# bilgili/Libre

Measured on AMD Instinct MI355X. Metric: Msamples/s + frames/s, 1024^3 volume @ 1024^2 viewport, higher is better.
Workload: dtype u8

## Files before the change

include/vrc_hip.h:

```cpp
#ifndef VRC_HIP_H
#define VRC_HIP_H

#include <stddef.h>
#include <stdint.h>

#ifdef __cplusplus
extern "C" {
#endif

#define VRC_OK 0
#define VRC_EINVAL 1
#define VRC_EHIP 2
#define VRC_EFULL 3
#define VRC_ENOMEM 4
#define VRC_EUNSUPPORTED 5
#define VRC_EHIERARCHY 6
#define VRC_ECOMM 7

typedef struct vrc_ctx vrc_ctx;
typedef struct vrc_pool vrc_pool;

typedef struct
{
    float textureMin[3];
// ... 76 lines not shown

#define VRC_OPT_RAY_CACHE 22
#define VRC_OPT_RAY_CACHE_USED 23

#define VRC_OPT_WALK_CACHE 24
#define VRC_WALK_CACHE_ALWAYS 2
#define VRC_OPT_WALK_CACHE_USED 25
#define VRC_OPT_WALK_CACHE_BUDGET 26
#define VRC_OPT_WALK_CACHE_BYTES 27
#define VRC_OPT_WALK_LEAN_USED 28
#define VRC_OPT_SHADING 29
#define VRC_OPT_SHADING_AMBIENT 30
#define VRC_OPT_COMPOSITE_DEPTH 31
#define VRC_OPT_PREINTEGRATION 32
#define VRC_OPT_PREINT_BUILDS 33
#define VRC_OPT_WALK_UNIFORM_ONLY 34
#define VRC_OPT_WALK_UNIFORM_ONLY_USED 35
#define VRC_OPT_STORE_THROUGH 36
#define VRC_OPT_STORE_THROUGH_USED 37
#define VRC_OPT_FIRST_VISIT_TABLE 38
#define VRC_OPT_FIRST_VISIT_TABLE_USED 39
#define VRC_OPT_LEAN_FREE_MARCH 40
#define VRC_OPT_LEAN_FREE_MARCH_USED 41
#define VRC_WALK_CACHE_DEFAULT_BUDGET ( 512ll << 20 )








#define VRC_VARIANT_CUDARAYCASTER 0
#define VRC_VARIANT_GLRAYCASTER 1

#define VRC_FILTER_NEAREST 0
#define VRC_FILTER_TRILINEAR 1

#define VRC_KERNEL_AUTO 0
#define VRC_REFERENCE_ORDER_MAX_NODES 4096
#define VRC_KERNEL_REFERENCE_ORDER 1
#define VRC_KERNEL_GRID_DDA 2
#define VRC_KERNEL_LDS 3
#define VRC_KERNEL_PACKED 5
#define VRC_KERNEL_RAY_LOD 4

// ... 90 lines not shown
```

libre_amd/csrc/vrc_api.hip:

```cpp
#include "../../include/vrc_hip.h"
#include "vrc_internal.h"
#include "vrc_plan.h"
#include "vrc_tables.h"

#include <algorithm>
#include <array>
#include <cmath>
#include <cstdarg>
#include <cstdio>
#include <cstring>
#include <memory>
#include <mutex>
#include <string>
#include <vector>

namespace
{
thread_local std::string g_lastError;

int fail( int code, const std::string& msg )
{
    g_lastError = msg;
    return code;
}
// ... 85 lines not shown

struct vrc_walk_cache
{
    enum { IDLE = 0, COUNTING = 1, VALID = 2 };
    int state = IDLE;
    uint32_t* dLists = nullptr;
    size_t words = 0;
    uint32_t k = 0;
    vrc_walk_count* dMax = nullptr;
    vrc_walk_count* hMax = nullptr;
    hipEvent_t ev = nullptr;
    vrc_frame frame;
    vrc_frame prevFrame;
    bool prevSet = false;
    uint64_t prevGen = 0, gen = 0;
    const uint32_t* slotInfo = nullptr;
    int64_t used = 0;
    bool leanAsked = false, lean = false;
    int64_t leanUsed = 0;
    unsigned long long gathers = 0;
    int64_t uniformUsed = 0;
    int64_t throughUsed = 0;
    int64_t freeUsed = 0;
};

struct vrc_first_visit
{
    void* dTable = nullptr;
    uint64_t gen = 0, prevGen = 0;
    bool grey = false;
    int64_t used = 0;
};

struct vrc_ctx
{
    int device = 0;
    hipStream_t ownStream = nullptr;
    hipStream_t stream = nullptr;
    vrc_options opt;
    vrc_latches latch;

    float* dTf = nullptr;
    float* hTf = nullptr;
    uint64_t tfVersion = 0;
    float planes[6][4];
    uint32_t nPlanes = 0;
// ... 225 lines not shown
        vrc_ctx_destroy( c );
        return fail( VRC_EHIP, msg );
    }
    c->stream = c->ownStream;
    *c->hCounter = 0;
    std::memcpy( c->hTf, tf, sizeof( tf ) );
    c->tfGrey = true;
    if( const char* g = std::getenv( "VRC_GREY_TABLE" ) )
        c->opt.greyTable = g[0] != '0';
    c->tfVersion = 1;
    *out = c;
    return VRC_OK;
}

void vrc_ctx_destroy( vrc_ctx* c )
{
    if( !c )
        return;
    (void)hipSetDevice( c->device );
    if( c->stream ) (void)hipStreamSynchronize( c->stream );
    const std::initializer_list< void* > device = {
        c->dTf,      c->dLut,     c->dPreint,  c->fbOwn,     c->dNodes,    c->dGrid,    c->dTileOrder, c->dRayCache,
        c->walk.dLists, c->walk.dMax, c->dRayList, c->dMipMax, c->dMeanSum, c->dMeanCount, c->dProjOut, c->dMipDepth,
        c->dIsoGrad, c->dDepthOut, c->dRowMap, c->dCounter,  c->dFrameHist, c->dHistRefs, c->first.dTable };
    const std::initializer_list< void* > pinned = { c->hTf, c->hStage, c->walk.hMax, c->hCounter, c->hFrameHist, c->hHistRefs };
    for( void* d : device )
        if( d ) (void)hipFree( d );
    for( void* h : pinned )
        if( h ) (void)hipHostFree( h );
    for( hipEvent_t e : c->stageEvent )
        if( e ) (void)hipEventDestroy( e );
    for( hipEvent_t e : c->histRefsEvent )
        if( e ) (void)hipEventDestroy( e );
    if( c->walk.ev ) (void)hipEventDestroy( c->walk.ev );
    c->evRing.reset();
    if( c->ownStream ) (void)hipStreamDestroy( c->ownStream );
    delete c;
}

int vrc_ctx_set_stream( vrc_ctx* c, void* s )
{
    if( !c )
        return fail( VRC_EINVAL, "vrc_ctx_set_stream: ctx is NULL" );
    VRC_HIP_CHECK( hipSetDevice( c->device ) );
    VRC_HIP_CHECK( hipStreamSynchronize( c->stream ) );
    c->stream = s ? (hipStream_t)s : c->ownStream;
    c->waitedPoolUid = c->waitedGen = 0;
// ... 59 lines not shown
    case VRC_OPT_WALK_UNIFORM_ONLY_USED:
        return fail( VRC_EINVAL, "vrc_set_option: VRC_OPT_WALK_UNIFORM_ONLY_USED is read-only" );
    case VRC_OPT_STORE_THROUGH:
        if( value != 0 && value != 1 )
            return fail( VRC_EINVAL, "vrc_set_option: VRC_OPT_STORE_THROUGH is 0 (plain stores) or 1 (write-through)" );
        c->opt.storeThrough = value;
        return VRC_OK;
    case VRC_OPT_STORE_THROUGH_USED:
        return fail( VRC_EINVAL, "vrc_set_option: VRC_OPT_STORE_THROUGH_USED is read-only" );
    case VRC_OPT_FIRST_VISIT_TABLE:
        if( value != 0 && value != 1 )
            return fail( VRC_EINVAL, "vrc_set_option: VRC_OPT_FIRST_VISIT_TABLE is 0 (march every visit) or 1 (first visits from the table)" );
        c->opt.firstVisitTable = value;
        return VRC_OK;
    case VRC_OPT_FIRST_VISIT_TABLE_USED:
        return fail( VRC_EINVAL, "vrc_set_option: VRC_OPT_FIRST_VISIT_TABLE_USED is read-only" );
    case VRC_OPT_LEAN_FREE_MARCH:
        if( value != 0 && value != 1 )
            return fail( VRC_EINVAL, "vrc_set_option: VRC_OPT_LEAN_FREE_MARCH is 0 (every visit tests for the exit) or 1 (not where it is out of reach)" );
        c->opt.leanFreeMarch = value;
        return VRC_OK;
    case VRC_OPT_LEAN_FREE_MARCH_USED:
        return fail( VRC_EINVAL, "vrc_set_option: VRC_OPT_LEAN_FREE_MARCH_USED is read-only" );
    case VRC_OPT_PROJECTION:
        if( value != VRC_PROJECTION_COMPOSITE && value != VRC_PROJECTION_MIP && value != VRC_PROJECTION_ISO )
            return fail( VRC_EINVAL, "vrc_set_option: VRC_OPT_PROJECTION is 0 (composite), 1 (maximum intensity) or 2 (isosurface)" );
        if( value == VRC_PROJECTION_ISO && !c->isoSet )
            return fail( VRC_EINVAL, "vrc_set_option: VRC_OPT_PROJECTION = VRC_PROJECTION_ISO needs vrc_set_isosurface first" );
        c->opt.projection = value;
        return VRC_OK;
    case VRC_OPT_MIP_SKIP: c->opt.mipSkip = value ? 1 : 0; return VRC_OK;
    case VRC_OPT_MIP_FOLD:
        if( value != VRC_MIP_FOLD_MAX && value != VRC_MIP_FOLD_MIN && value != VRC_MIP_FOLD_MEAN )
            return fail( VRC_EINVAL, "vrc_set_option: VRC_OPT_MIP_FOLD is 0 (maximum), 1 (minimum) or 2 (mean)" );
        c->opt.mipFold = value;
        return VRC_OK;
    case VRC_OPT_MIP_DEPTH:
        if( value != 0 && value != 1 )
            return fail( VRC_EINVAL, "vrc_set_option: VRC_OPT_MIP_DEPTH is 0 (off) or 1 (keep the depth of the projected sample)" );
        c->opt.mipDepth = value;
        return VRC_OK;
    case VRC_OPT_MIP_DEPTH_CUE:
        if( value < 0 || value > 1000 )
            return fail( VRC_EINVAL, "vrc_set_option: VRC_OPT_MIP_DEPTH_CUE is the cue strength in thousandths, 0 (off) to 1000" );
        c->opt.mipDepthCue = value;
        return VRC_OK;
// ... 48 lines not shown
    case VRC_OPT_STEPPING: *value = c->opt.stepping; return VRC_OK;
    case VRC_OPT_KERNEL_TIMING: *value = c->opt.timing; return VRC_OK;
    case VRC_OPT_DEPTH_SPLIT: *value = c->opt.depthSplit; return VRC_OK;
    case VRC_OPT_ERT_COMPACTION: *value = c->opt.ertParts; return VRC_OK;
    case VRC_OPT_GREY_TABLE: *value = c->opt.greyTable; return VRC_OK;
    case VRC_OPT_PACKED_ATLAS: *value = c->opt.packedAtlas; return VRC_OK;
    case VRC_OPT_UNIFORM_BRICKS: *value = c->opt.uniformBricks; return VRC_OK;
    case VRC_OPT_STREAM_MARKERS: *value = c->opt.streamMarkers; return VRC_OK;
    case VRC_OPT_RAY_CACHE: *value = c->opt.rayCache; return VRC_OK;
    case VRC_OPT_RAY_CACHE_USED: *value = c->rayCacheUsed; return VRC_OK;
    case VRC_OPT_WALK_CACHE: *value = c->opt.walkCache; return VRC_OK;
    case VRC_OPT_WALK_CACHE_USED: *value = c->walk.used; return VRC_OK;
    case VRC_OPT_WALK_CACHE_BUDGET: *value = c->opt.walkBudget; return VRC_OK;
    case VRC_OPT_WALK_CACHE_BYTES: *value = (int64_t)( c->walk.words * sizeof( uint32_t ) ); return VRC_OK;
    case VRC_OPT_WALK_LEAN_USED: *value = c->walk.leanUsed; return VRC_OK;
    case VRC_OPT_WALK_UNIFORM_ONLY: *value = c->opt.walkUniformOnly; return VRC_OK;
    case VRC_OPT_WALK_UNIFORM_ONLY_USED: *value = c->walk.uniformUsed; return VRC_OK;
    case VRC_OPT_STORE_THROUGH: *value = c->opt.storeThrough; return VRC_OK;
    case VRC_OPT_STORE_THROUGH_USED: *value = c->walk.throughUsed; return VRC_OK;
    case VRC_OPT_FIRST_VISIT_TABLE: *value = c->opt.firstVisitTable; return VRC_OK;
    case VRC_OPT_FIRST_VISIT_TABLE_USED: *value = c->first.used; return VRC_OK;
    case VRC_OPT_LEAN_FREE_MARCH: *value = c->opt.leanFreeMarch; return VRC_OK;
    case VRC_OPT_LEAN_FREE_MARCH_USED: *value = c->walk.freeUsed; return VRC_OK;
    case VRC_OPT_PROJECTION: *value = c->opt.projection; return VRC_OK;
    case VRC_OPT_MIP_SKIP: *value = c->opt.mipSkip; return VRC_OK;
    case VRC_OPT_MIP_FOLD: *value = c->opt.mipFold; return VRC_OK;
    case VRC_OPT_MIP_DEPTH: *value = c->opt.mipDepth; return VRC_OK;
    case VRC_OPT_MIP_DEPTH_CUE: *value = c->opt.mipDepthCue; return VRC_OK;
    case VRC_OPT_VARIANT: *value = c->opt.variant; return VRC_OK;
    case VRC_OPT_SHADING: *value = c->opt.shading; return VRC_OK;
    case VRC_OPT_SHADING_AMBIENT: *value = c->opt.shadingAmbient; return VRC_OK;
    case VRC_OPT_COMPOSITE_DEPTH: *value = c->opt.compositeDepth; return VRC_OK;
    case VRC_OPT_PREINTEGRATION: *value = c->opt.preint; return VRC_OK;
    case VRC_OPT_PREINT_BUILDS: *value = c->preintBuilds; return VRC_OK;
    case VRC_OPT_KERNEL_USED: *value = c->stats.kernel_variant; return VRC_OK;
    case VRC_OPT_GRID_WALK_USED: *value = c->gridWalkUsed; return VRC_OK;
    default: return fail( VRC_EINVAL, "vrc_get_option: unknown option" );
    }
}

int vrc_set_ray_lod( vrc_ctx* c, int enable, float screenSpaceError, float worldSpacePerPixel )
{
    if( !c )
        return fail( VRC_EINVAL, "vrc_set_ray_lod: ctx is NULL" );
    if( enable && ( !( screenSpaceError > 0.0f ) || !( worldSpacePerPixel > 0.0f ) ) )
        return fail( VRC_EINVAL, "vrc_set_ray_lod: screen-space error and world space per pixel must be > 0" );
// ... 855 lines not shown
{
    if( !c )
        return fail( VRC_EINVAL, "vrc_get_framebuffer: ctx is NULL" );
    VRC_TRY( resolve_clear( c ) );
    if( deviceRgba ) *deviceRgba = ctx_fb( c );
    if( width ) *width = c->fbW;
    if( height ) *height = c->fbH;
    return VRC_OK;
}

struct render_pass
{
    const vrc_view_data* view;
    const vrc_node_data* nodes;
    uint32_t nNodes;
    const vrc_render_data* render;
    vrc_pool* pool;
    vrc_lut_params lp;
    vrc_mode mode;
    vrc_form form;
    bool sameNodes, tableWalk;
    size_t pixels, plane;
    bool walkCount, walkRecord;
    vrc_raycast_args a;
};

static int render_check_args( vrc_ctx* c, const vrc_view_data* view, const vrc_node_data* nodes, uint32_t nNodes,
                              const vrc_render_data* render, vrc_pool* pool )
{
    if( !c || !view || !render || !pool )
        return fail( VRC_EINVAL, "vrc_render: NULL argument" );
    if( nNodes > 0 && !nodes )
        return fail( VRC_EINVAL, "vrc_render: nodes is NULL" );
    if( pool->device != c->device )
        return fail( VRC_EINVAL, "vrc_render: pool lives on another device" );
    if( !ctx_fb( c ) || c->fbW == 0 )
        return fail( VRC_EINVAL, "vrc_render: vrc_pre_render has not been called" );
    if( view->glViewport[2] != c->fbW ||
        ( c->rowMap.empty() ? view->glViewport[3] : (uint32_t)c->rowMap.size() ) != c->fbH )
        return fail( VRC_EINVAL, "vrc_render: viewport differs from the pixel buffer" );
    if( render->samplesPerRay == 0 )
        return fail( VRC_EINVAL, "vrc_render: samplesPerRay is 0" );
    if( render->dataSourceRange[1] == render->dataSourceRange[0] )
        return fail( VRC_EINVAL, "vrc_render: empty data source range" );
    return VRC_OK;
}
// ... 487 lines not shown
    }
    else if( p.walkCount )
        f.walkLean = leanAsked ? 1u : 0u;
    w.throughUsed = vrc_plan_store_through( c->opt, w.used, f.width, f.height ) ? 1 : 0;
    f.storeThrough = (uint32_t)w.throughUsed;
    vrc_first_visit& fv = c->first;
    const bool grey = p.a.greyTable;
    vrc_first_visit_facts k = { w.used, f.walkLean, f.clearFirst != 0u, p.mode.classify,
                                fv.gen != 0u && fv.gen == c->lutGen && fv.grey == grey };
    if( vrc_plan_first_visit_build( c->opt, k, fv.prevGen == c->lutGen ) )
    {
        if( !fv.dTable )
            VRC_HIP_CHECK( hipMalloc( &fv.dTable, (size_t)VRC_FIRST_VISIT_ENTRIES * VRC_FIRST_VISIT_ROWS * sizeof( vrc_f4 ) ) );
        VRC_HIP_CHECK( vrc_launch_build_first_visit( c->dLut, fv.dTable, grey, c->stream ) );
        fv.gen = c->lutGen;
        fv.grey = grey;
        k.current = true;
    }
    fv.prevGen = c->lutGen;
    fv.used = vrc_plan_first_visit( c->opt, k ) ? 1 : 0;
    f.firstVisit = fv.used ? fv.dTable : nullptr;
    w.freeUsed = vrc_plan_lean_free_march( c->opt, w.used, f.walkLean, p.mode.classify ) ? 1 : 0;
    f.leanFree = (uint32_t)w.freeUsed;
    return VRC_OK;
}

static int render_march( vrc_ctx* c, render_pass& p )
{
    vrc_raycast_args& a = p.a;
    vrc_frame& f = a.frame;
    const vrc_mode& m = p.mode;
    VRC_TRY( ctx_wait_uploads( c, p.pool ) );
    if( p.walkCount )
    {
        VRC_HIP_CHECK( hipMemsetAsync( c->walk.dMax, 0, sizeof( vrc_walk_count ), c->stream ) );
        VRC_HIP_CHECK( vrc_launch_walk_record( a, c->walk.dMax, c->stream ) );
        VRC_HIP_CHECK( hipMemcpyAsync( c->walk.hMax, c->walk.dMax, sizeof( vrc_walk_count ), hipMemcpyDeviceToHost, c->stream ) );
        VRC_HIP_CHECK( hipEventRecord( c->walk.ev, c->stream ) );
        std::memcpy( &c->walk.frame, &f, sizeof( f ) );
        c->walk.state = vrc_walk_cache::COUNTING;
        f.walkLean = 0u;
    }
    if( p.walkRecord )
    {
        VRC_HIP_CHECK( vrc_launch_walk_record( a, nullptr, c->stream ) );
        c->walk.state = vrc_walk_cache::VALID;
        f.walkCache = nullptr;
        f.walkPlane = f.walkK = 0u;
        f.walkLean = f.walkSlots = 0u;
    }
    if( c->opt.count )
        VRC_HIP_CHECK( hipMemsetAsync( c->dCounter, 0, sizeof( unsigned long long ), c->stream ) );
    if( c->opt.timing && c->evUsed == c->evRing->pairs.size() )
    {
        if( c->evRing->pairs.size() >= 4096 )
        {
            VRC_HIP_CHECK( hipEventSynchronize( c->evRing->pairs[c->evUsed - 1].second ) );
            for( size_t i = 0; i < c->evUsed; ++i )
            {
                float ms = 0.f;
                VRC_HIP_CHECK( hipEventElapsedTime( &ms, c->evRing->pairs[i].first, c->evRing->pairs[i].second ) );
                c->evFoldedMs += ms;
            }
            c->evFoldedLaunches += (uint32_t)c->evUsed;
            c->evUsed = 0;
        }
        else
        {
            hipEvent_t a0 = nullptr, a1 = nullptr;
            VRC_HIP_CHECK( hipEventCreate( &a0 ) );
            VRC_HIP_CHECK( hipEventCreate( &a1 ) );
            c->evRing->pairs.push_back( { a0, a1 } );
// ... 346 lines not shown
```

libre_amd/csrc/vrc_core.h:

```cpp
#ifndef VRC_CORE_H
#define VRC_CORE_H

#if !defined( VRC_DEV_BUILD ) && ( \
    defined( VRC_ABLATE_NO_FETCH ) || \
    defined( VRC_WG_TIMELINE ) || \
    defined( VRC_UNIFORM_GROUP ) || \
    defined( VRC_LEAN_GROUP ) || defined( VRC_LEAN_FREE_GROUP ) || \
    defined( VRC_TEST_BIAS_ENTRY ) || \
    defined( VRC_LDS_STATS ) || defined( VRC_LDS_STATS2 ) || \
    defined( VRC_LDS_TIMING ) || \
    defined( VRC_LDS_PASSES ) || defined( VRC_LDS_ROWS ) || defined( VRC_LDS_OCC ) || defined( VRC_LDS_STAGE_N ) || \
    defined( VRC_LDS_ROWS16 ) || defined( VRC_LDS_OCC16 ) || defined( VRC_LDS_STAGE_N16 ) || \
    defined( VRC_LDS_KMAX ) || \
    defined( VRC_LDS_MAX_DZ ) || \
    defined( VRC_LDS_LBATCH ) || \
    defined( VRC_LDS_GBATCH ) || \
    defined( VRC_LDS_G ) || defined( VRC_LDS_GF ) || \
    defined( VRC_LDS_WAVES ) || \
    defined( VRC_LDS_REFILL ) || defined( VRC_LDS_SOON ) || \
    defined( VRC_GROUP ) || \
    defined( VRC_GREY_GROUP ) || \
    defined( VRC_GREY_MAX_WAVES ) || defined( VRC_REPLAY_GREY_MAX_WAVES ) || \
    defined( VRC_REPLAY_UNIFORM_MAX_WAVES ) || defined( VRC_REPLAY_UNIFORM_WG_WAVES ) || \
    defined( VRC_LGROUP ) || \
// ... 111 lines not shown
    uint32_t* meanCount;
    float* mipDepth;
    float mipCue;
    float* rayCache;
    uint32_t rayCachePlane;
    uint32_t rayMode;
    float* isoGrad;
    uint32_t isoThreshold;
    float isoStored;
    float isoClassify;
    float isoAmbient;
    uint32_t* walkCache;
    uint32_t walkPlane;
    uint32_t walkK;
#define VRC_WALK_LEAN_UNIFORM 2u
    uint32_t walkLean;
    uint32_t walkSlots;
    float shadeAmbient;
    float cdepthTau;
    const vrc_f4* preintTable;
    uint32_t storeThrough;
    const void* firstVisit;
    uint32_t leanFree;
};
#define VRC_RAY_COMPUTE 0u
#define VRC_RAY_STORE 1u
#define VRC_RAY_LOAD 2u
#define VRC_RAY_CACHE_PLANES 10u

struct vrc_layout
{
    uint32_t slots[3];
    uint32_t slotDim[3];
};

VRC_HD uint32_t vrc_mb_y( uint32_t u ) { return ( ( u & 3u ) << 3 ) | ( ( u & 4u ) << 5 ); }
VRC_HD uint32_t vrc_mb_z( uint32_t u ) { return ( ( u & 3u ) << 5 ) | ( ( u & 4u ) << 6 ); }
#define VRC_MB_FIX_Y( u ) ( 96u * ( ( ( u ) >> 2 ) & 1u ) )
#define VRC_MB_FIX_Z( u ) ( 32u * ( ( u ) & 3u ) )
struct vrc_lay
{
    uint32_t a, b, c;
};
VRC_HD vrc_lay vrc_make_lay( uint32_t sbx, uint32_t sby )
{
    vrc_lay l;
// ... 4118 lines not shown
VRC_HD vrc_f4 vrc_lean_narrow( const vrc_f4& c, const vrc_f4* ) { return c; }
VRC_HD vrc_f4 vrc_lean_widen( const vrc_f2& c ) { return vrc_f4{ c.x, c.x, c.x, c.w }; }
VRC_HD vrc_f4 vrc_lean_widen( const vrc_f4& c ) { return c; }
VRC_HD uint32_t vrc_lean_slot_load( const vrc_frame& f, uint32_t packed )
{
    const uint32_t idx = packed & ( ( 1u << VRC_WALK_LEAN_INDEX_BITS ) - 1u );
    const bool have = f.slotInfo != nullptr;
    const uint32_t* const from = have ? f.slotInfo : f.walkCache;
    const uint32_t last = have ? f.walkSlots - 1u : 0u;
    const uint32_t i = idx != 0u ? idx - 1u : 0u;
    return from[i < last ? i : last];
}
VRC_HD uint32_t vrc_lean_slot_word( const vrc_frame& f, uint32_t packed, uint32_t loaded )
{
    return ( f.slotInfo != nullptr && ( packed & ( ( 1u << VRC_WALK_LEAN_INDEX_BITS ) - 1u ) ) != 0u ) ? loaded : 0u;
}
VRC_HD uint32_t vrc_lean_list_word( const vrc_frame& f, uint32_t rayIndex, uint32_t v )
{
    const uint32_t lastVisit = f.walkK - 1u;
    const size_t plane = 2u + 4u * (size_t)( v < lastVisit ? v : lastVisit );
    return f.walkCache[(size_t)rayIndex + plane * f.walkPlane];
}

template < bool COUNT, int MODE, int GROUP, bool UNIFORM_ONLY = false >
VRC_HD void vrc_pixel_walk_replay_lean( const vrc_frame& f, const vrc_dev_node* __restrict__ nodes,
                                        const uint8_t* __restrict__ atlas, const vrc_f4* lut, const vrc_classifier& cls,
                                        vrc_f4* __restrict__ pixelBuffer, uint32_t px, uint32_t py, uint32_t& nSamples,
                                        uint32_t rayIndex )
{
    typedef typename vrc_lean_colour< MODE >::type E;
    (void)cls;
    const E* const tab = reinterpret_cast< const E* >( lut );
    const uint32_t pixelPos = py * f.width + px;
    const vrc_f4 zero = { 0.f, 0.f, 0.f, 0.f };
    const uint32_t listed = f.walkCache[rayIndex];
    const uint32_t count = listed < f.walkK ? listed : f.walkK;
    if( count == 0u )
    {
        if( f.clearFirst )
            vrc_store_pixel( f, pixelBuffer, pixelPos, zero );
        return;
    }
    const vrc_f4 start = f.clearFirst ? zero : pixelBuffer[pixelPos];
    if( start.w > VRC_EARLY_EXIT )
        return;
    E color = vrc_lean_narrow( start, (const E*)nullptr );
    const uint32_t lastNode = f.nodeCount - 1u;
    const bool freeMarch = f.leanFree != 0u;
    uint32_t packed = vrc_lean_list_word( f, rayIndex, 0u );
    uint32_t packedNext = vrc_lean_list_word( f, rayIndex, 1u );
    uint32_t loaded = vrc_lean_slot_load( f, packed );
    uint32_t k = 0u;
    bool ended = false;
    if constexpr( !COUNT )
// ... 456 lines not shown
```

libre_amd/csrc/vrc_internal.h:

```cpp
#ifndef VRC_INTERNAL_H
#define VRC_INTERNAL_H

#include <hip/hip_runtime.h>
#include <hip/hip_ext.h>
#include <stdint.h>

#include "vrc_core.h"

#ifndef VRC_TILE_W
#define VRC_TILE_W 8u
#endif
#define VRC_TILE_H ( 64u / VRC_TILE_W )

#define VRC_NO_TILE 0xFFFFFFFFu
#define VRC_WAVES_PER_GROUP 4u
#ifndef VRC_SUPER_UNITS
#define VRC_SUPER_UNITS 1u
#endif
#define VRC_XCDS 8u
__host__ __device__ inline uint32_t vrc_super_x( uint32_t tilesX ) { return ( ( tilesX + 1u ) / 2u + VRC_SUPER_UNITS - 1u ) / VRC_SUPER_UNITS; }
__host__ __device__ inline uint32_t vrc_schedule_units( uint32_t tilesX, uint32_t tilesY )
{
    const uint32_t nSuper = vrc_super_x( tilesX ) * vrc_super_x( tilesY );
    return ( nSuper + VRC_XCDS - 1u ) / VRC_XCDS * VRC_XCDS * VRC_SUPER_UNITS * VRC_SUPER_UNITS;
// ... 111 lines not shown
#endif
#ifndef VRC_SMALL_GROUP
#define VRC_SMALL_GROUP 24
#endif
#ifndef VRC_SMALL_LAUNCH_TILES
#define VRC_SMALL_LAUNCH_TILES 6144u
#endif
static inline bool vrc_walk_replay_eligible( const vrc_raycast_args& a )
{
    return a.gridDda && a.gridTable && !a.packed && !a.linear && a.elemBytes == 1 && !a.bigAtlas && !a.clamp &&
           a.fixedStepping && a.ertParts <= 1 && !a.depthSplit && !a.shade && !a.cdepth && !a.preint && VRC_TILE_W == 8u;
}
static inline int vrc_walk_replay_group( const vrc_raycast_args& a )
{
    const uint32_t tiles = ( ( a.frame.width + VRC_TILE_W - 1 ) / VRC_TILE_W ) * ( ( a.frame.height + VRC_TILE_H - 1 ) / VRC_TILE_H );
    return tiles <= VRC_SMALL_LAUNCH_TILES ? VRC_SMALL_GROUP : ( a.greyTable ? VRC_GREY_GROUP : VRC_GROUP );
}
struct vrc_walk_count
{
    uint32_t longest, notLean;
    unsigned long long visits, gathers;
};
hipError_t vrc_launch_walk_record( const vrc_raycast_args& a, vrc_walk_count* result, hipStream_t stream );
hipError_t vrc_launch_raycast_replay( const vrc_raycast_args& a, hipStream_t stream );

hipError_t vrc_launch_raycast_mip( const vrc_raycast_args& a, hipStream_t stream );
hipError_t vrc_launch_raycast_minip( const vrc_raycast_args& a, hipStream_t stream );
hipError_t vrc_launch_raycast_meanip( const vrc_raycast_args& a, hipStream_t stream );

struct vrc_projection_state
{
    const uint32_t* mipMax;
    const unsigned long long* meanSum;
    const uint32_t* meanCount;
    uint32_t pixels;
    uint32_t fold;
    uint32_t floatState;
    float shift;
};
hipError_t vrc_launch_projection_values( const vrc_projection_state& st, float* values, uint32_t* counts, hipStream_t stream );

hipError_t vrc_launch_raycast_mip_depth( const vrc_raycast_args& a, int fold, hipStream_t stream );
hipError_t vrc_launch_projection_depths( const vrc_frame& f, const float* depth, uint32_t pixels, float* t, float* xyz,
                                         hipStream_t stream );

hipError_t vrc_launch_raycast_iso( const vrc_raycast_args& a, hipStream_t stream );
// ... 23 lines not shown
```

libre_amd/csrc/vrc_kernels_walk.hip:

```cpp
#include "vrc_internal.h"

#define VRC_WALK_WAVES VRC_WAVES_PER_GROUP
#define VRC_WALK_THREADS ( 64u * VRC_WALK_WAVES )

__device__ inline void vrc_walk_lane_pixel( uint32_t tile, uint32_t tilesX, uint32_t lane, uint32_t& px, uint32_t& py )
{
    const uint32_t tx = tile % tilesX, ty = tile / tilesX;
    const uint32_t lx = ( lane & 1u ) | ( ( lane >> 1 ) & 2u ) | ( ( lane >> 2 ) & 4u );
    const uint32_t ly = ( ( lane >> 1 ) & 1u ) | ( ( lane >> 2 ) & 2u ) | ( ( lane >> 3 ) & 4u );
    px = tx * 8u + lx;
    py = ty * 8u + ly;
}

__global__ __launch_bounds__( VRC_WALK_THREADS ) void vrc_k_walk_record(
    const vrc_frame f, const vrc_dev_node* __restrict__ nodes, const int32_t* __restrict__ gridTable,
    vrc_walk_count* __restrict__ result, const uint32_t tilesX, const uint32_t nTiles )
{
    const uint32_t lane = threadIdx.x & 63u;
    const uint32_t tile = blockIdx.x * VRC_WALK_WAVES + ( threadIdx.x >> 6 );
    if( tile >= nTiles )
        return;
    uint32_t px, py;
    vrc_walk_lane_pixel( tile, tilesX, lane, px, py );
    const uint32_t rayIndex = tile * 64u + lane;
// ... 38 lines not shown
                        0, stream, a.frame, a.nodes, a.gridTable, result, tilesX, nTiles );
    return hipGetLastError();
}

template < typename E >
__global__ __launch_bounds__( 64 ) void vrc_k_build_first_visit( const vrc_f4* __restrict__ lut, E* __restrict__ table, const E start )
{
    const uint32_t e = blockIdx.x * 64u + threadIdx.x;
    if( e < VRC_FIRST_VISIT_ENTRIES )
        vrc_first_visit_row< E >( table + (size_t)e * VRC_FIRST_VISIT_ROWS, vrc_lean_narrow( lut[e], (const E*)nullptr ), start );
}

hipError_t vrc_launch_build_first_visit( const vrc_f4* lut, void* table, bool grey, hipStream_t stream )
{
    if( !lut || !table )
        return hipErrorInvalidValue;
    const dim3 grid( ( VRC_FIRST_VISIT_ENTRIES + 63u ) / 64u ), block( 64 );
    if( grey )
        hipLaunchKernelGGL( vrc_k_build_first_visit< vrc_f2 >, grid, block, 0, stream, lut, static_cast< vrc_f2* >( table ),
                            vrc_f2{ 0.f, 0.f } );
    else
        hipLaunchKernelGGL( vrc_k_build_first_visit< vrc_f4 >, grid, block, 0, stream, lut, static_cast< vrc_f4* >( table ),
                            vrc_f4{ 0.f, 0.f, 0.f, 0.f } );
    return hipGetLastError();
}

#ifndef VRC_REPLAY_GREY_MAX_WAVES
#define VRC_REPLAY_GREY_MAX_WAVES 6
#endif
#ifndef VRC_REPLAY_UNIFORM_MAX_WAVES
#define VRC_REPLAY_UNIFORM_MAX_WAVES 8
#endif
#ifndef VRC_REPLAY_UNIFORM_WG_WAVES
#define VRC_REPLAY_UNIFORM_WG_WAVES VRC_WALK_WAVES
#endif
#define VRC_REPLAY_K_MIN_WAVES ( UNIFORM ? VRC_REPLAY_UNIFORM_MAX_WAVES : ( GROUP > VRC_GREY_GROUP ? 2 : 5 ) )
#define VRC_REPLAY_K_MAX_WAVES \
    ( UNIFORM ? VRC_REPLAY_UNIFORM_MAX_WAVES \
              : ( GROUP > VRC_GREY_GROUP ? 8 : ( MODE == VRC_MODE_GREY ? VRC_REPLAY_GREY_MAX_WAVES : 5 ) ) )
#define VRC_REPLAY_K_WAVES ( UNIFORM ? VRC_REPLAY_UNIFORM_WG_WAVES : VRC_WALK_WAVES )
template < bool COUNT, int MODE, int GROUP, bool LEAN = false, bool UNIFORM = false >
__global__ __launch_bounds__( 64u * VRC_REPLAY_K_WAVES ) __attribute__( ( amdgpu_waves_per_eu( VRC_REPLAY_K_MIN_WAVES, VRC_REPLAY_K_MAX_WAVES ) ) ) void vrc_k_raycast_replay(
    const vrc_frame f, const vrc_dev_node* __restrict__ nodes, const uint8_t* __restrict__ atlas,
    const vrc_f4* __restrict__ lutGlobal, const vrc_classifier cls, vrc_f4* __restrict__ pixelBuffer,
    unsigned long long* __restrict__ sampleCounter, const uint32_t* __restrict__ tileOrder, const uint32_t tilesX,
    const uint32_t nTiles )
// ... 9 lines not shown
        vrc_f2* const lut2 = reinterpret_cast< vrc_f2* >( lut );
        for( uint32_t i = tid; i < VRC_LUT_ENTRIES; i += THREADS )
        {
            const vrc_f4 e = lutGlobal[i];
            lut2[i] = vrc_f2{ e.x, e.w };
        }
    }
    else
    {
        for( uint32_t i = tid; i < VRC_TFP_ENTRIES; i += THREADS )
            lut[i] = lutGlobal[i];
    }
    if constexpr( !UNIFORM )
    {
        const vrc_lay lay = vrc_make_lay( f.sbx, f.sby );
        for( uint32_t u = tid; u < 256u; u += THREADS )
        {
            vrc_addr_tab[u] = vrc_lay_x( lay, u );
            vrc_addr_tab[256u + u] = vrc_lay_y( lay, u );
            vrc_addr_tab[512u + u] = vrc_lay_z( lay, u );
        }
    }
    __syncthreads();
    const uint32_t slotIndex = blockIdx.x * WAVES + ( tid >> 6 );
    const uint32_t tilesY = nTiles / tilesX;
    if( slotIndex >= vrc_schedule_slots( tilesX, tilesY ) )
        return;
    const uint32_t tile = vrc_slot_tile( tileOrder, slotIndex, tilesX, tilesY );
    if( tile == VRC_NO_TILE )
        return;
    uint32_t px, py;
    vrc_walk_lane_pixel( tile, tilesX, lane, px, py );

    uint32_t nSamples = 0;
    if( px < f.width && py < f.height )
    {
        if constexpr( LEAN )
            vrc_pixel_walk_replay_lean< COUNT, MODE, GROUP, UNIFORM >( f, nodes, atlas, lut, cls, pixelBuffer, px, py,
                                                                       nSamples, tile * 64u + lane );
        else
            vrc_pixel_walk_replay< COUNT, MODE, GROUP >( f, nodes, atlas, lut, cls, pixelBuffer, px, py, nSamples,
                                                         tile * 64u + lane );
    }
    if( COUNT )
    {
        unsigned long long s = nSamples;
#pragma unroll
        for( int off = 32; off > 0; off >>= 1 )
            s += __shfl_down( s, off, 64 );
        if( lane == 0 && s != 0 )
            atomicAdd( sampleCounter, s );
    }
}

template < bool COUNT, int MODE, int GROUP, bool LEAN, bool UNIFORM = false >
// ... 43 lines not shown
```

libre_amd/csrc/vrc_plan.h:

```cpp
#ifndef VRC_PLAN_H
#define VRC_PLAN_H

#include "../../include/vrc_hip.h"

struct vrc_options
{
    int64_t kernel = VRC_KERNEL_AUTO, variant = VRC_VARIANT_CUDARAYCASTER;
    int64_t filter = 0, tfFracBits = 8, stepping = 1;
    int64_t count = 0, timing = 1, streamMarkers = 0;
    int64_t depthSplit = 0, ertParts = 0;
    int64_t packedAtlas = 1, uniformBricks = 1, greyTable = 1, tileOrder = 1, rayCache = 1;
    int64_t walkCache = 1, walkBudget = VRC_WALK_CACHE_DEFAULT_BUDGET, walkUniformOnly = 1;
    int64_t projection = VRC_PROJECTION_COMPOSITE, mipSkip = 1, mipFold = VRC_MIP_FOLD_MAX;
    int64_t mipDepth = 0, mipDepthCue = 0;
    int64_t shading = 0, shadingAmbient = 250;
    int64_t compositeDepth = 0, preint = 0;
    int64_t storeThrough = 1;
    int64_t firstVisitTable = 1;
    int64_t leanFreeMarch = 1;
};

struct vrc_latches
{
    int64_t projection = -1, fold = -1, depth = -1, cue = -1;
    bool iso = false;
    float isoValue = 0.0f, isoAmbient = 0.0f;
    int64_t shading = -1, shadingAmbient = -1, compositeDepth = -1, preint = -1;
};

struct vrc_refusal
{
    int code;
    const char* msg;
};

struct vrc_mode
{
    bool iso = false, mip = false;
    bool mipDepth = false, mean = false;
    bool shade = false, cdepth = false, preint = false;
    bool linear = false;
    bool classify = false;
// ... 203 lines not shown
    uint32_t walkLean;
    bool clearFirst;
    bool classify;
    bool current;
};
inline bool vrc_plan_first_visit_wanted( const vrc_options& o, const vrc_first_visit_facts& k )
{
    return o.firstVisitTable != 0 && k.walkUsed == 4 && k.walkLean != 0u && k.clearFirst && !k.classify && o.count == 0;
}
inline bool vrc_plan_first_visit( const vrc_options& o, const vrc_first_visit_facts& k )
{
    return vrc_plan_first_visit_wanted( o, k ) && k.current;
}
inline bool vrc_plan_first_visit_build( const vrc_options& o, const vrc_first_visit_facts& k, bool prevSameGeneration )
{
    return vrc_plan_first_visit_wanted( o, k ) && !k.current && prevSameGeneration;
}

inline bool vrc_plan_lean_free_march( const vrc_options& o, int64_t walkUsed, uint32_t walkLean, bool classify )
{
    return o.leanFreeMarch != 0 && walkUsed == 4 && walkLean != 0u && !classify && o.count == 0;
}

#endif
```

libre_amd/vrc.py:

```python
import ctypes as C
import os

_HERE = os.path.dirname(os.path.abspath(__file__))
LIB_PATH = os.path.join(_HERE, "lib", "libvrc_hip.so")

VRC_OK, VRC_EINVAL, VRC_EHIP, VRC_EFULL, VRC_ENOMEM, VRC_EUNSUPPORTED, VRC_EHIERARCHY, VRC_ECOMM = range(8)
OPT_KERNEL, OPT_FILTER, OPT_TF_FRAC_BITS, OPT_COUNT_SAMPLES, OPT_TILE_ORDER, OPT_STEPPING, OPT_VARIANT, OPT_KERNEL_USED, OPT_KERNEL_TIMING, OPT_DEPTH_SPLIT, OPT_ERT_COMPACTION, OPT_GREY_TABLE, OPT_PACKED_ATLAS, OPT_GRID_WALK_USED, OPT_UNIFORM_BRICKS = range(1, 16)
OPT_PROJECTION, OPT_MIP_SKIP, OPT_MIP_FOLD = 16, 17, 18
OPT_MIP_DEPTH, OPT_MIP_DEPTH_CUE = 19, 20
OPT_STREAM_MARKERS = 21
OPT_RAY_CACHE, OPT_RAY_CACHE_USED = 22, 23
OPT_WALK_CACHE, OPT_WALK_CACHE_USED, OPT_WALK_CACHE_BUDGET, OPT_WALK_CACHE_BYTES = 24, 25, 26, 27
WALK_CACHE_ALWAYS = 2
OPT_WALK_LEAN_USED = 28
OPT_SHADING, OPT_SHADING_AMBIENT = 29, 30
OPT_COMPOSITE_DEPTH = 31
OPT_PREINTEGRATION = 32
OPT_PREINT_BUILDS = 33
OPT_WALK_UNIFORM_ONLY, OPT_WALK_UNIFORM_ONLY_USED = 34, 35
OPT_STORE_THROUGH, OPT_STORE_THROUGH_USED = 36, 37
OPT_FIRST_VISIT_TABLE, OPT_FIRST_VISIT_TABLE_USED = 38, 39
OPT_LEAN_FREE_MARCH, OPT_LEAN_FREE_MARCH_USED = 40, 41
PREINT_VALUE, PREINT_TEXEL = 0, 1
PROJECTION_COMPOSITE, PROJECTION_MIP, PROJECTION_ISO = 0, 1, 2
MIP_FOLD_MAX, MIP_FOLD_MIN, MIP_FOLD_MEAN = 0, 1, 2
VARIANT_CUDARAYCASTER, VARIANT_GLRAYCASTER = 0, 1
FILTER_NEAREST, FILTER_TRILINEAR = 0, 1
KERNEL_AUTO, KERNEL_REFERENCE_ORDER, KERNEL_GRID_DDA, KERNEL_LDS, KERNEL_RAY_LOD, KERNEL_PACKED = 0, 1, 2, 3, 4, 5

VOXEL_UINT8, VOXEL_UINT16, VOXEL_UINT32, VOXEL_INT8, VOXEL_INT16, VOXEL_INT32, VOXEL_FLOAT32 = range(7)

ABI_VERSION = 4

f32x3 = C.c_float * 3
u32x3 = C.c_uint32 * 3


class NodeData(C.Structure):
    _fields_ = [("textureMin", f32x3), ("textureSize", f32x3),
                ("aabbMin", f32x3), ("aabbSize", f32x3)]


class ViewData(C.Structure):
    _fields_ = [("eyePosition", f32x3), ("glViewport", C.c_uint32 * 4),
                ("invProjMatrix", C.c_float * 16), ("modelViewMatrix", C.c_float * 16),
# ... 156 lines not shown
```

Baseline: 14.20 million.

## Precompute resolved per-visit walk words for uniform-only lean replay

Adds a resolve kernel that, once per walk-cache generation, folds each ray's list word and slot-info lookup into a single resolved word (sample count, one-value flag, value byte). The uniform-only lean replay then reads these words directly with prefetching, which removes the indirect slot-table loads and dependent address math from the per-frame replay. Tile and slot indices are also made wave-uniform through readfirstlane. The cost is an extra device buffer of K words per pixel, a one-time resolve pass, and invalidation bookkeeping tied to generation and slot info.

```diff
diff --git a/include/vrc_hip.h b/include/vrc_hip.h
--- a/include/vrc_hip.h
+++ b/include/vrc_hip.h
@@ -122,6 +122,8 @@
 #define VRC_OPT_FIRST_VISIT_TABLE_USED 39
 #define VRC_OPT_LEAN_FREE_MARCH 40
 #define VRC_OPT_LEAN_FREE_MARCH_USED 41
+#define VRC_OPT_WALK_RESOLVED 42
+#define VRC_OPT_WALK_RESOLVED_USED 43
 #define VRC_WALK_CACHE_DEFAULT_BUDGET ( 512ll << 20 )
 
 
diff --git a/libre_amd/csrc/vrc_api.hip b/libre_amd/csrc/vrc_api.hip
--- a/libre_amd/csrc/vrc_api.hip
+++ b/libre_amd/csrc/vrc_api.hip
@@ -131,6 +131,12 @@
     int64_t uniformUsed = 0;
     int64_t throughUsed = 0;
     int64_t freeUsed = 0;
+    uint32_t* dResolved = nullptr;
+    size_t resolvedWords = 0;
+    bool resolvedValid = false;
+    uint64_t resolvedGen = 0;
+    const uint32_t* resolvedSlotInfo = nullptr;
+    int64_t resolvedUsed = 0;
 };
 
 struct vrc_first_visit
@@ -402,7 +408,8 @@
     const std::initializer_list< void* > device = {
         c->dTf,      c->dLut,     c->dPreint,  c->fbOwn,     c->dNodes,    c->dGrid,    c->dTileOrder, c->dRayCache,
         c->walk.dLists, c->walk.dMax, c->dRayList, c->dMipMax, c->dMeanSum, c->dMeanCount, c->dProjOut, c->dMipDepth,
-        c->dIsoGrad, c->dDepthOut, c->dRowMap, c->dCounter,  c->dFrameHist, c->dHistRefs, c->first.dTable };
+        c->dIsoGrad, c->dDepthOut, c->dRowMap, c->dCounter,  c->dFrameHist, c->dHistRefs, c->first.dTable,
+        c->walk.dResolved };
     const std::initializer_list< void* > pinned = { c->hTf, c->hStage, c->walk.hMax, c->hCounter, c->hFrameHist, c->hHistRefs };
     for( void* d : device )
         if( d ) (void)hipFree( d );
@@ -508,6 +515,13 @@
         return VRC_OK;
     case VRC_OPT_LEAN_FREE_MARCH_USED:
         return fail( VRC_EINVAL, "vrc_set_option: VRC_OPT_LEAN_FREE_MARCH_USED is read-only" );
+    case VRC_OPT_WALK_RESOLVED:
+        if( value != 0 && value != 1 )
+            return fail( VRC_EINVAL, "vrc_set_option: VRC_OPT_WALK_RESOLVED is 0 (list and slot words) or 1 (resolved visit words)" );
+        c->opt.walkResolved = value;
+        return VRC_OK;
+    case VRC_OPT_WALK_RESOLVED_USED:
+        return fail( VRC_EINVAL, "vrc_set_option: VRC_OPT_WALK_RESOLVED_USED is read-only" );
     case VRC_OPT_PROJECTION:
         if( value != VRC_PROJECTION_COMPOSITE && value != VRC_PROJECTION_MIP && value != VRC_PROJECTION_ISO )
             return fail( VRC_EINVAL, "vrc_set_option: VRC_OPT_PROJECTION is 0 (composite), 1 (maximum intensity) or 2 (isosurface)" );
@@ -602,6 +616,8 @@
     case VRC_OPT_FIRST_VISIT_TABLE_USED: *value = c->first.used; return VRC_OK;
     case VRC_OPT_LEAN_FREE_MARCH: *value = c->opt.leanFreeMarch; return VRC_OK;
     case VRC_OPT_LEAN_FREE_MARCH_USED: *value = c->walk.freeUsed; return VRC_OK;
+    case VRC_OPT_WALK_RESOLVED: *value = c->opt.walkResolved; return VRC_OK;
+    case VRC_OPT_WALK_RESOLVED_USED: *value = c->walk.resolvedUsed; return VRC_OK;
     case VRC_OPT_PROJECTION: *value = c->opt.projection; return VRC_OK;
     case VRC_OPT_MIP_SKIP: *value = c->opt.mipSkip; return VRC_OK;
     case VRC_OPT_MIP_FOLD: *value = c->opt.mipFold; return VRC_OK;
@@ -1503,6 +1519,7 @@
     bool sameNodes, tableWalk;
     size_t pixels, plane;
     bool walkCount, walkRecord;
+    bool walkResolve;
     vrc_raycast_args a;
 };
 
@@ -2036,6 +2053,21 @@
     f.firstVisit = fv.used ? fv.dTable : nullptr;
     w.freeUsed = vrc_plan_lean_free_march( c->opt, w.used, f.walkLean, p.mode.classify ) ? 1 : 0;
     f.leanFree = (uint32_t)w.freeUsed;
+    p.walkResolve = false;
+    const bool uniformOnly = f.walkLean == VRC_WALK_LEAN_UNIFORM;
+    if( w.resolvedValid && ( p.walkRecord || ( w.used == 4 && ( w.resolvedGen != gen || w.resolvedSlotInfo != f.slotInfo ) ) ) )
+        w.resolvedValid = false;
+    const unsigned long long resolvedBytes = ( 1ull + 5ull * w.k ) * plane * sizeof( uint32_t );
+    w.resolvedUsed = vrc_plan_walk_resolved( c->opt, uniformOnly, resolvedBytes <= (unsigned long long)c->opt.walkBudget ) ? 1 : 0;
+    if( w.resolvedUsed && !w.resolvedValid )
+    {
+        const size_t words = (size_t)w.k * plane;
+        VRC_TRY( ctx_grow( c, w.resolvedWords, words, words, { w.dResolved } ) );
+        p.walkResolve = true;
+        w.resolvedGen = gen;
+        w.resolvedSlotInfo = f.slotInfo;
+    }
+    f.walkResolved = w.resolvedUsed ? w.dResolved : nullptr;
     return VRC_OK;
 }
 
@@ -2062,6 +2094,11 @@
         f.walkCache = nullptr;
         f.walkPlane = f.walkK = 0u;
         f.walkLean = f.walkSlots = 0u;
+    }
+    if( p.walkResolve )
+    {
+        VRC_HIP_CHECK( vrc_launch_walk_resolve( f, c->walk.dResolved, c->stream ) );
+        c->walk.resolvedValid = true;
     }
     if( c->opt.count )
         VRC_HIP_CHECK( hipMemsetAsync( c->dCounter, 0, sizeof( unsigned long long ), c->stream ) );
diff --git a/libre_amd/csrc/vrc_core.h b/libre_amd/csrc/vrc_core.h
--- a/libre_amd/csrc/vrc_core.h
+++ b/libre_amd/csrc/vrc_core.h
@@ -157,6 +157,7 @@
     uint32_t storeThrough;
     const void* firstVisit;
     uint32_t leanFree;
+    const uint32_t* walkResolved;
 };
 #define VRC_RAY_COMPUTE 0u
 #define VRC_RAY_STORE 1u
@@ -4321,6 +4322,92 @@
     return f.walkCache[(size_t)rayIndex + plane * f.walkPlane];
 }
 
+VRC_HD void vrc_replay_tile_origin( uint32_t tile, uint32_t tilesX, uint32_t& x0, uint32_t& y0 )
+{
+    const uint32_t ty = tile / tilesX;
+    x0 = ( tile - ty * tilesX ) * 8u;
+    y0 = ty * 8u;
+}
+VRC_HD void vrc_replay_lane_pixel( uint32_t x0, uint32_t y0, uint32_t lane, uint32_t& px, uint32_t& py )
+{
+    px = x0 + ( ( lane & 1u ) | ( ( lane >> 1 ) & 2u ) | ( ( lane >> 2 ) & 4u ) );
+    py = y0 + ( ( ( lane >> 1 ) & 1u ) | ( ( lane >> 2 ) & 2u ) | ( ( lane >> 3 ) & 4u ) );
+}
+
+#define VRC_WALK_RESOLVED_ONE 0x100u
+VRC_HD uint32_t vrc_walk_resolved_word( const vrc_frame& f, uint32_t rayIndex, uint32_t v )
+{
+    const uint32_t listed = f.walkCache[rayIndex];
+    const uint32_t packed = vrc_lean_list_word( f, rayIndex, v );
+    const uint32_t word = vrc_lean_slot_word( f, packed, vrc_lean_slot_load( f, packed ) );
+    const uint32_t one = ( v < listed && vrc_slot_holds_one_value( word ) ) ? VRC_WALK_RESOLVED_ONE : 0u;
+    return ( packed & ~( ( 1u << VRC_WALK_LEAN_INDEX_BITS ) - 1u ) ) | one | ( word & 0xFFu );
+}
+VRC_HD uint32_t vrc_walk_resolved_load( const vrc_frame& f, uint32_t rayIndex, uint32_t v )
+{
+    const uint32_t lastVisit = f.walkK - 1u;
+    return f.walkResolved[(size_t)rayIndex + (size_t)( v < lastVisit ? v : lastVisit ) * f.walkPlane];
+}
+
+template < int MODE >
+VRC_HD void vrc_pixel_walk_replay_resolved( const vrc_frame& f, const vrc_f4* lut, vrc_f4* __restrict__ pixelBuffer,
+                                            uint32_t px, uint32_t py, uint32_t rayIndex )
+{
+    typedef typename vrc_lean_colour< MODE >::type E;
+    const E* const tab = reinterpret_cast< const E* >( lut );
+    const uint32_t pixelPos = py * f.width + px;
+    const vrc_f4 zero = { 0.f, 0.f, 0.f, 0.f };
+    uint32_t listed = f.walkCache[rayIndex];
+    uint32_t res = vrc_walk_resolved_load( f, rayIndex, 0u );
+    uint32_t resNext = vrc_walk_resolved_load( f, rayIndex, 1u );
+#if defined( __HIP_DEVICE_COMPILE__ )
+    asm volatile( "" : "+v"( listed ), "+v"( res ), "+v"( resNext ) );
+#endif
+    if( listed == 0u )
+    {
+        if( f.clearFirst )
+            vrc_store_pixel( f, pixelBuffer, pixelPos, zero );
+        return;
+    }
+    const vrc_f4 start = f.clearFirst ? zero : pixelBuffer[pixelPos];
+    if( start.w > VRC_EARLY_EXIT )
+        return;
+    E color = vrc_lean_narrow( start, (const E*)nullptr );
+    const bool freeMarch = f.leanFree != 0u;
+    const uint32_t K = f.walkK;
+    uint32_t nSamples = 0u;
+    uint32_t k = 0u;
+    const E* const first = static_cast< const E* >( f.firstVisit );
+    if( first != nullptr && f.clearFirst )
+    {
+        const uint32_t resAfter = vrc_walk_resolved_load( f, rayIndex, 2u );
+        const uint32_t n = res >> VRC_WALK_LEAN_INDEX_BITS;
+        const bool one = ( res & VRC_WALK_RESOLVED_ONE ) != 0u;
+        bool done = true;
+        if( one && n < VRC_FIRST_VISIT_ROWS )
+        {
+            color = first[( res & 0xFFu ) * VRC_FIRST_VISIT_ROWS + n];
+            done = color.w > VRC_EARLY_EXIT;
+        }
+        else if( one )
+            done = vrc_march_uniform_lean< false, E >( color, tab[res & 0xFFu], n, nSamples, freeMarch );
+        res = done ? 0u : resNext;
+        resNext = resAfter;
+        k = 1u;
+    }
+    for( ; k < K; ++k )
+    {
+        const uint32_t resAfter = vrc_walk_resolved_load( f, rayIndex, k + 2u );
+        if( ( res & VRC_WALK_RESOLVED_ONE ) == 0u )
+            break;
+        if( vrc_march_uniform_lean< false, E >( color, tab[res & 0xFFu], res >> VRC_WALK_LEAN_INDEX_BITS, nSamples, freeMarch ) )
+            break;
+        res = resNext;
+        resNext = resAfter;
+    }
+    vrc_store_pixel( f, pixelBuffer, pixelPos, vrc_lean_widen( color ) );
+}
+
 template < bool COUNT, int MODE, int GROUP, bool UNIFORM_ONLY = false >
 VRC_HD void vrc_pixel_walk_replay_lean( const vrc_frame& f, const vrc_dev_node* __restrict__ nodes,
                                         const uint8_t* __restrict__ atlas, const vrc_f4* lut, const vrc_classifier& cls,
@@ -4329,6 +4416,14 @@
 {
     typedef typename vrc_lean_colour< MODE >::type E;
     (void)cls;
+    if constexpr( UNIFORM_ONLY && !COUNT )
+    {
+        if( f.walkResolved != nullptr )
+        {
+            vrc_pixel_walk_replay_resolved< MODE >( f, lut, pixelBuffer, px, py, rayIndex );
+            return;
+        }
+    }
     const E* const tab = reinterpret_cast< const E* >( lut );
     const uint32_t pixelPos = py * f.width + px;
     const vrc_f4 zero = { 0.f, 0.f, 0.f, 0.f };
diff --git a/libre_amd/csrc/vrc_internal.h b/libre_amd/csrc/vrc_internal.h
--- a/libre_amd/csrc/vrc_internal.h
+++ b/libre_amd/csrc/vrc_internal.h
@@ -157,6 +157,7 @@
     unsigned long long visits, gathers;
 };
 hipError_t vrc_launch_walk_record( const vrc_raycast_args& a, vrc_walk_count* result, hipStream_t stream );
+hipError_t vrc_launch_walk_resolve( const vrc_frame& f, uint32_t* resolved, hipStream_t stream );
 hipError_t vrc_launch_raycast_replay( const vrc_raycast_args& a, hipStream_t stream );
 
 hipError_t vrc_launch_raycast_mip( const vrc_raycast_args& a, hipStream_t stream );
diff --git a/libre_amd/csrc/vrc_kernels_walk.hip b/libre_amd/csrc/vrc_kernels_walk.hip
--- a/libre_amd/csrc/vrc_kernels_walk.hip
+++ b/libre_amd/csrc/vrc_kernels_walk.hip
@@ -84,6 +84,23 @@
     else
         hipLaunchKernelGGL( vrc_k_build_first_visit< vrc_f4 >, grid, block, 0, stream, lut, static_cast< vrc_f4* >( table ),
                             vrc_f4{ 0.f, 0.f, 0.f, 0.f } );
+    return hipGetLastError();
+}
+
+__global__ __launch_bounds__( 256 ) void vrc_k_walk_resolve( const vrc_frame f, uint32_t* __restrict__ resolved )
+{
+    const uint32_t rayIndex = blockIdx.x * 256u + threadIdx.x;
+    if( rayIndex >= f.walkPlane )
+        return;
+    for( uint32_t v = 0u; v < f.walkK; ++v )
+        resolved[(size_t)rayIndex + (size_t)v * f.walkPlane] = vrc_walk_resolved_word( f, rayIndex, v );
+}
+
+hipError_t vrc_launch_walk_resolve( const vrc_frame& f, uint32_t* resolved, hipStream_t stream )
+{
+    if( !resolved || !f.walkCache || f.walkK == 0u || f.walkPlane == 0u || f.walkLean == 0u || f.walkSlots == 0u )
+        return hipErrorInvalidValue;
+    hipLaunchKernelGGL( vrc_k_walk_resolve, dim3( ( f.walkPlane + 255u ) / 256u ), dim3( 256 ), 0, stream, f, resolved );
     return hipGetLastError();
 }
 
@@ -139,15 +156,16 @@
         }
     }
     __syncthreads();
-    const uint32_t slotIndex = blockIdx.x * WAVES + ( tid >> 6 );
+    const uint32_t slotIndex = __builtin_amdgcn_readfirstlane( blockIdx.x * WAVES + ( tid >> 6 ) );
     const uint32_t tilesY = nTiles / tilesX;
     if( slotIndex >= vrc_schedule_slots( tilesX, tilesY ) )
         return;
-    const uint32_t tile = vrc_slot_tile( tileOrder, slotIndex, tilesX, tilesY );
+    const uint32_t tile = __builtin_amdgcn_readfirstlane( vrc_slot_tile( tileOrder, slotIndex, tilesX, tilesY ) );
     if( tile == VRC_NO_TILE )
         return;
-    uint32_t px, py;
-    vrc_walk_lane_pixel( tile, tilesX, lane, px, py );
+    uint32_t x0, y0, px, py;
+    vrc_replay_tile_origin( tile, tilesX, x0, y0 );
+    vrc_replay_lane_pixel( x0, y0, lane, px, py );
 
     uint32_t nSamples = 0;
     if( px < f.width && py < f.height )
diff --git a/libre_amd/csrc/vrc_plan.h b/libre_amd/csrc/vrc_plan.h
--- a/libre_amd/csrc/vrc_plan.h
+++ b/libre_amd/csrc/vrc_plan.h
@@ -18,6 +18,7 @@
     int64_t storeThrough = 1;
     int64_t firstVisitTable = 1;
     int64_t leanFreeMarch = 1;
+    int64_t walkResolved = 1;
 };
 
 struct vrc_latches
@@ -267,4 +268,9 @@
     return o.leanFreeMarch != 0 && walkUsed == 4 && walkLean != 0u && !classify && o.count == 0;
 }
 
+inline bool vrc_plan_walk_resolved( const vrc_options& o, bool uniformOnly, bool fits )
+{
+    return o.walkResolved != 0 && uniformOnly && fits && o.count == 0;
+}
+
 #endif
diff --git a/libre_amd/vrc.py b/libre_amd/vrc.py
--- a/libre_amd/vrc.py
+++ b/libre_amd/vrc.py
@@ -21,6 +21,7 @@
 OPT_STORE_THROUGH, OPT_STORE_THROUGH_USED = 36, 37
 OPT_FIRST_VISIT_TABLE, OPT_FIRST_VISIT_TABLE_USED = 38, 39
 OPT_LEAN_FREE_MARCH, OPT_LEAN_FREE_MARCH_USED = 40, 41
+OPT_WALK_RESOLVED, OPT_WALK_RESOLVED_USED = 42, 43
 PREINT_VALUE, PREINT_TEXEL = 0, 1
 PROJECTION_COMPOSITE, PROJECTION_MIP, PROJECTION_ISO = 0, 1, 2
 MIP_FOLD_MAX, MIP_FOLD_MIN, MIP_FOLD_MEAN = 0, 1, 2
```

Result: faster. 15.19 million (median of 6 runs) (+6.9%).
